# Vchitect/Latte

Hardware: AMD Instinct MI355X
Metric: denoising steps/sec (higher is better)
Workload: dtype f16; 1 GPU; Latte-XL/2 FaceForensics (uncond) 16x256x256 -> latents 16x4x32x32, DDIM on the '250' respacing, random-init weights; per_gpu_batch=8, global_batch=8, parallelism=dp1 (independent samples)

## Files before the change

### include/latte_amd_debug.h

```cpp
#ifndef LATTE_AMD_DEBUG_H_
#define LATTE_AMD_DEBUG_H_
#include <stdint.h>
#ifdef __cplusplus
extern "C" {
#endif

int latte_debug_gemm(const void* A, const void* W, const float* bias, void* out, const float* gate, int M, int N,
                     int K, int gate_stride, int rows_per_sample, int epi, int dtype, int variant, void* stream);
int latte_debug_gemm_gelu(const void* A, const void* W, const float* bias, void* out, void* aux, int M, int N, int K, int epi, int dtype,
                          void* stream);
int latte_debug_gemm_lo8(const void* A, const void* W, const void* A8, const void* W8, const float* bias, void* out, const float* gate,
                         int M, int N, int K, int gate_stride, int rows_per_sample, int epi, int dtype, void* stream);
int latte_debug_pack_w8(const void* w, void* out8, int64_t n, int dtype, void* stream);
int latte_debug_pack_w4(const void* w, void* out4, void* out_scale, int N, int K, int dtype, void* stream);
int latte_debug_ln_modulate_split4(const float* x, void* y, void* y4, void* y4s, const float* shift, const float* scale, int mod_stride, int M,
                                   int D, int rows_per_sample, int dtype, void* stream);
int latte_debug_gemm_lo4(const void* A, const void* W, const void* A4, const void* A4s, const void* W4, const void* W4s, const float* bias,
                         void* out, const float* gate, int M, int N, int K, int gate_stride, int rows_per_sample, int epi, int dtype,
                         void* stream);
int latte_debug_ln_modulate_split8(const float* x, void* y, void* y8, const float* shift, const float* scale, int mod_stride, int M, int D,
                                   int rows_per_sample, int dtype, void* stream);
int latte_debug_qkv_attention_split8(const void* xn, const void* w, const float* bias, void* out, void* out8, int B, int F, int T, int D,
                                     int heads, int mode, int dtype, void* stream);
int latte_debug_gemm_choice(int M, int N, int K, int epi);
int latte_debug_qkv_attention_fusable(int D, int heads, int F, int T, int mode, int64_t rows);
int latte_debug_gemm_tn_plan(int M, int N, int K, int* rows_per_split);
int latte_debug_attention(const void* qkv, void* out, int num_seq, int L, int heads, int hd, int U,
                          int64_t sample_stride, int64_t seq_stride, int64_t row_stride, int dtype, void* stream);
int latte_debug_cross_attention(const void* q, int q_ld, const void* kv, const float* kbias_or_null, void* out, int num_seq, int L, int Lk,
                                int heads, int hd, int U, int64_t sample_stride, int64_t seq_stride, int64_t row_stride, int dtype,
                                void* stream);
int latte_debug_small_linear(int in_mode, const float* in, const int64_t* t, const float* W, const float* bias, const float* add_table,
                             const int64_t* add_idx, float* out, int B, int N, int K, int out_stride, void* stream);
int latte_debug_patch_embed(const float* x, const float* Wt, const float* bias, const float* pos, float* out, int BF, int C, int H, int p,
                            int D, void* stream);
int latte_debug_final_layer(const float* x, const float* shift, const float* scale, int mod_stride, const float* Wt, const float* bias,
                            float* out, int M, int D, int rows_per_sample, int T, int p, int Cout, int H, void* stream);
int latte_debug_text_proj(const float* text, const float* W, const float* bias, float* out, int B, int N, int K, void* stream);
int latte_debug_gated_split_reduce(float* x, const float* ws, int splits, int64_t stride, const float* bias, const float* gate,
                                   int gate_stride, int rows_per_sample, int M, int N, void* stream);
int latte_debug_adaln_single(const float* tables, const float* head_table, const float* t6, const float* temb, float* mod, int B, int nblk,
                             int D, void* stream);
int latte_debug_cond_rows(const float* temb, const float* ytab, const int64_t* y, float* out, int n_steps, int bu, int D, void* stream);
int latte_debug_mask_bias(const float* mask, float* bias, int64_t n, void* stream);
int latte_debug_t2v_linear_step(float* x, float* x_in, const float* model_out, const float* h1, const float* h2, const float* h3,
                                const float* noise, float* hist_write, int b, int C, int Cout, int F, int hw, float scale, float m_x,
                                float m_eps, float c_x, float c0, float c1, float c2, float c3, float c_noise, float in_scale_next,
                                int push, void* stream);
int latte_debug_attention_split8(const void* qkv, void* out, void* out8, int num_seq, int L, int heads, int hd, int U, int64_t sample_stride,
                                 int64_t seq_stride, int64_t row_stride, int dtype, void* stream);
int latte_debug_qkv_attention(const void* xn, const void* w, const float* bias, void* out, void* dbg_qkv, int B, int F, int T,
                              int D, int heads, int mode, int flags, int dtype, void* stream);
int latte_debug_qkv_attention_trace(const void* xn, const void* w, const float* bias, void* out, void* dbg_qkv, long long* trace,
                                    int B, int F, int T, int D, int heads, int mode, int flags, int dtype, void* stream);
int latte_debug_attention_bwd(const void* qkv, const void* o, const void* dout, void* dqkv, float* stats, int num_seq, int L,
                              int heads, int hd, int U, int64_t sample_stride, int64_t seq_stride, int64_t row_stride, int dtype,
                              void* stream);
int latte_debug_gemm_tn(const void* dY, const void* X, float* dW, float* workspace, int64_t workspace_floats, int M, int N, int K,
                        int dtype, void* stream);
int latte_debug_gemm_tn_colsum(const void* dY, const void* X, float* dW, float* colsum, float* workspace, int64_t workspace_floats,
                               int M, int N, int K, int dtype, void* stream);
int latte_debug_ln_modulate(float* x, void* y, const float* shift, const float* scale, int mod_stride, int M, int D,
                            int rows_per_sample, const float* temp_embed, int T, int F, int dtype, void* stream);
int latte_debug_convert(const float* in, void* out, int64_t n, int dtype, void* stream);
int latte_debug_gated_add_ln(const float* x_in, const void* y, const float* gate, int gate_stride, float* x_out, void* xn,
                             const float* shift, const float* scale, int mod_stride, int M, int D, int rows_per_sample,
                             const float* temp_embed, int T, int F, int dtype, void* stream);
int latte_debug_ln_bwd(const void* dy, const float* x, const float* scale, int mod_stride, const float* dx_in, float* dx_out,
// ... 113 lines not shown
```

### latte_amd/_lib.py

```python
import ctypes
import os

import torch

_HERE = os.path.dirname(os.path.abspath(__file__))
LIB_PATH = os.path.join(_HERE, "lib", "liblatte_amd.so")

c_int, c_i64, c_f32, c_void, c_char = ctypes.c_int, ctypes.c_int64, ctypes.c_float, ctypes.c_void_p, ctypes.c_char_p
c_u64 = ctypes.c_uint64


class LatteError(RuntimeError):
    pass


class ModelConfig(ctypes.Structure):
    _fields_ = [(n, c_int) for n in ("input_size", "patch_size", "in_channels", "hidden_size", "depth", "num_heads",
                                     "mlp_hidden", "num_frames", "num_classes", "learn_sigma", "extras",
                                     "compute_dtype")]


class T2VConfig(ctypes.Structure):
    _fields_ = [(n, c_int) for n in ("num_attention_heads", "attention_head_dim", "in_channels", "out_channels", "num_layers",
                                     "sample_size", "patch_size", "cross_attention_dim", "caption_channels", "video_length",
# ... 110 lines not shown
    "latte_debug_t5_embed": (c_int, [c_void, c_void, c_void, c_int, c_int, c_int, c_void]),
    "latte_debug_t5_rmsnorm": (c_int, [c_void, c_void, c_void, c_void, c_void, c_int, c_int, c_f32, c_void]),
    "latte_debug_t5_bucket": (c_int, [c_int, c_int, c_int]),
    "latte_debug_t5_bias_table": (c_int, [c_void, c_int, c_int, c_int, c_int, c_void, c_void]),
    "latte_debug_t5_attention": (c_int, [c_void, c_void, c_void, c_void, c_void, c_int, c_int, c_int, c_int, c_void]),
    "latte_debug_t5_gated_act": (c_int, [c_void, c_void, c_void, c_int, c_int, c_void]),
    "latte_debug_t5_pack": (c_int, [c_void, c_void, c_void, c_i64, c_void]),
    "latte_debug_t5_proj_splits": (c_int, [c_int, c_int]),
    "latte_debug_t5_proj": (c_int, [c_void, c_void, c_void, c_void, c_void, c_void, c_int, c_int, c_int, c_void]),
    "latte_debug_gemm_lo8": (c_int, [c_void, c_void, c_void, c_void, c_void, c_void, c_void, c_int, c_int, c_int, c_int, c_int, c_int,
                                     c_int, c_void]),
    "latte_debug_attention_split8": (c_int, [c_void, c_void, c_void, c_int, c_int, c_int, c_int, c_int, c_i64, c_i64, c_i64, c_int, c_void]),
    "latte_debug_pack_w4": (c_int, [c_void, c_void, c_void, c_int, c_int, c_int, c_void]),
    "latte_debug_ln_modulate_split4": (c_int, [c_void, c_void, c_void, c_void, c_void, c_void, c_int, c_int, c_int, c_int, c_int, c_void]),
    "latte_debug_gemm_lo4": (c_int, [c_void, c_void, c_void, c_void, c_void, c_void, c_void, c_void, c_void, c_int, c_int, c_int, c_int, c_int,
                                     c_int, c_int, c_void]),
    "latte_debug_pack_w8": (c_int, [c_void, c_void, c_i64, c_int, c_void]),
    "latte_debug_ln_modulate_split8": (c_int, [c_void, c_void, c_void, c_void, c_void, c_int, c_int, c_int, c_int, c_int, c_void]),
    "latte_debug_qkv_attention_split8": (c_int, [c_void, c_void, c_void, c_void, c_void, c_int, c_int, c_int, c_int, c_int, c_int, c_int,
                                                 c_void]),
    "latte_debug_gemm": (c_int, [c_void, c_void, c_void, c_void, c_void, c_int, c_int, c_int, c_int, c_int, c_int,
                                 c_int, c_int, c_void]),
    "latte_debug_gemm_gelu": (c_int, [c_void, c_void, c_void, c_void, c_void, c_int, c_int, c_int, c_int, c_int, c_void]),
    "latte_debug_gemm_choice": (c_int, [c_int, c_int, c_int, c_int]),
    "latte_debug_qkv_attention_fusable": (c_int, [c_int, c_int, c_int, c_int, c_int, c_i64]),
    "latte_debug_gemm_tn_plan": (c_int, [c_int, c_int, c_int, ctypes.POINTER(c_int)]),
    "latte_debug_attention": (c_int, [c_void, c_void, c_int, c_int, c_int, c_int, c_int, c_i64, c_i64, c_i64, c_int,
                                      c_void]),
    "latte_debug_cross_attention": (c_int, [c_void, c_int, c_void, c_void, c_void, c_int, c_int, c_int, c_int, c_int, c_int, c_i64, c_i64,
                                            c_i64, c_int, c_void]),
    "latte_debug_small_linear": (c_int, [c_int, c_void, c_void, c_void, c_void, c_void, c_void, c_void, c_int, c_int, c_int, c_int,
                                         c_void]),
    "latte_debug_patch_embed": (c_int, [c_void, c_void, c_void, c_void, c_void, c_int, c_int, c_int, c_int, c_int, c_void]),
    "latte_debug_final_layer": (c_int, [c_void, c_void, c_void, c_int, c_void, c_void, c_void, c_int, c_int, c_int, c_int, c_int, c_int,
                                        c_int, c_void]),
    "latte_debug_text_proj": (c_int, [c_void, c_void, c_void, c_void, c_int, c_int, c_int, c_void]),
    "latte_debug_gated_split_reduce": (c_int, [c_void, c_void, c_int, c_i64, c_void, c_void, c_int, c_int, c_int, c_int, c_void]),
    "latte_debug_adaln_single": (c_int, [c_void, c_void, c_void, c_void, c_void, c_int, c_int, c_int, c_void]),
    "latte_debug_cond_rows": (c_int, [c_void, c_void, c_void, c_void, c_int, c_int, c_int, c_void]),
    "latte_debug_mask_bias": (c_int, [c_void, c_void, c_i64, c_void]),
    "latte_debug_t2v_linear_step": (c_int, [c_void] * 8 + [c_int] * 5 + [c_f32] * 10 + [c_int, c_void]),
    "latte_debug_qkv_attention": (c_int, [c_void, c_void, c_void, c_void, c_void, c_int, c_int, c_int, c_int, c_int, c_int, c_int,
                                          c_int, c_void]),
    "latte_debug_qkv_attention_trace": (c_int, [c_void, c_void, c_void, c_void, c_void, c_void, c_int, c_int, c_int, c_int, c_int,
                                                c_int, c_int, c_int, c_void]),
    "latte_debug_attention_bwd": (c_int, [c_void, c_void, c_void, c_void, c_void, c_int, c_int, c_int, c_int, c_int, c_i64, c_i64, c_i64,
                                          c_int, c_void]),
    "latte_debug_gemm_tn": (c_int, [c_void, c_void, c_void, c_void, c_i64, c_int, c_int, c_int, c_int, c_void]),
    "latte_debug_gemm_tn_colsum": (c_int, [c_void, c_void, c_void, c_void, c_void, c_i64, c_int, c_int, c_int, c_int, c_void]),
    "latte_debug_ln_modulate": (c_int, [c_void, c_void, c_void, c_void, c_int, c_int, c_int, c_int, c_void, c_int,
                                        c_int, c_int, c_void]),
    "latte_debug_convert": (c_int, [c_void, c_void, c_i64, c_int, c_void]),
    "latte_debug_gated_add_ln": (c_int, [c_void, c_void, c_void, c_int, c_void, c_void, c_void, c_void, c_int, c_int, c_int, c_int,
                                         c_void, c_int, c_int, c_int, c_void]),
    "latte_debug_ln_bwd": (c_int, [c_void, c_void, c_void, c_int, c_void, c_void, c_void, c_void, c_int, c_int, c_int, c_int, c_void,
                                   c_void, c_int, c_void, c_void, c_void, c_i64, c_int, c_void]),
    "latte_debug_gate_bwd": (c_int, [c_void, c_void, c_void, c_int, c_void, c_void, c_i64, c_void, c_int, c_int, c_int, c_int, c_int,
                                     c_int, c_void]),
    "latte_debug_split_reduce": (c_int, [c_void, c_int, c_i64, c_i64, c_void, c_int, c_void, c_void]),
    "latte_debug_colsum_half": (c_int, [c_void, c_int, c_int, c_void, c_i64, c_void, c_int, c_int, c_void, c_void]),
    "latte_debug_rows_sum": (c_int, [c_void, c_int, c_i64, c_int, c_void, c_int, c_void, c_void]),
    "latte_debug_naive_gemm": (c_int, [c_void, c_i64, c_i64, c_void, c_i64, c_i64, c_void, c_i64, c_i64, c_int, c_int, c_int, c_f32,
                                       c_int, c_int, c_void, c_i64, c_void, c_void]),
    "latte_debug_embedding_bwd": (c_int, [c_void, c_void, c_void, c_int, c_int, c_void, c_void]),
    "latte_debug_silu_bwd": (c_int, [c_void, c_void, c_void, c_i64, c_int, c_void]),
    "latte_debug_sumsq_blocks": (c_int, []),
# ... 125 lines not shown
```

### latte_amd/csrc/common.h

```cpp
#pragma once
#include <hip/hip_runtime.h>
#include <stdint.h>
#include <atomic>
#include <string>
#include <vector>

#include "../../include/latte_amd.h"

struct latte_schedule {
  int num_timesteps = 0;
  std::vector<int64_t> timestep_map;
  std::vector<double> betas, alphas_cumprod, alphas_cumprod_prev, sqrt_recip_alphas_cumprod,
      sqrt_recipm1_alphas_cumprod, posterior_variance, posterior_log_variance_clipped, posterior_mean_coef1,
      posterior_mean_coef2, log_betas, sqrt_alphas_cumprod, sqrt_one_minus_alphas_cumprod;
  int mean_type = 0;
  int var_type = 0;
  mutable float* dev_tables = nullptr;
  mutable int dev_tables_device = -1;
};
enum DevTable : int { DT_SQRT_AC = 0, DT_SQRT_1MAC, DT_COEF1, DT_COEF2, DT_POST_LOGVAR, DT_LOG_BETAS, DT_SQRT_RECIP, DT_SQRT_RECIPM1,
                      DT_FIXED_LOGVAR, LATTE_NUM_DEV_TABLES };

extern "C" int schedule_device_tables(const latte_schedule_t* s, const float** out, hipStream_t st);

// ... 101 lines not shown
int launch_attention(const AttnArgs& a, int dtype, hipStream_t st);
int launch_cross_attention(const AttnArgs& a, int dtype, hipStream_t st);

struct QkvAttnArgs {
  const half_t* xn;
  const half_t* w;
  const float* bias;
  half_t* out;
  half_t* dbg_qkv;
  long long* dbg_trace;
  int B, F, T, D, heads, hd;
  int mode;
  float scale;
  int flags;
  int out_split;
  unsigned char* out8;
};
bool qkv_attention_fusable(int D, int heads, int hd, int F, int T, int mode, int64_t rows);
int launch_qkv_attention(const QkvAttnArgs& a, int dtype, hipStream_t st);

int launch_ln_modulate_split4(const float* x_in, half_t* y, unsigned char* y4, unsigned char* y4s, const float* shift, const float* scale,
                              int mod_stride, int M, int D, int rows_per_sample, int dtype, hipStream_t st);
int launch_ln_modulate(const float* x_in, float* x_rw, half_t* y, const float* shift, const float* scale,
                       int mod_stride, int M, int D, int rows_per_sample, const float* temp_embed, int T,
                       int F, int dtype, hipStream_t st, int split = 0,
                       unsigned char* y8 = nullptr);
int launch_pack_w8(const half_t* in, unsigned char* out, int64_t n, int dtype, hipStream_t st);
enum SmallIn : int { IN_PLAIN = 0, IN_SILU = 1, IN_TFREQ = 2 };
int launch_small_linear(int in_mode, const float* in, const int64_t* t, const float* W, const float* bias,
                        const float* add_table, const int64_t* add_idx, float* out, int B, int N, int K,
                        int out_stride, hipStream_t st);
int launch_patch_embed(const float* x, const float* Wt , const float* bias, const float* pos,
                       float* out, int BF, int C, int H, int p, int D, hipStream_t st);
int launch_final_layer(const float* x, const float* shift, const float* scale, int mod_stride,
                       const float* Wt , const float* bias, float* out, int M, int D,
                       int rows_per_sample, int T, int p, int Cout, int H, hipStream_t st);
int launch_cond_rows(const float* temb, const float* ytab, const int64_t* y, float* out, int n_steps, int bu, int D,
                     hipStream_t st);
int launch_text_proj(const float* text, const float* W, const float* bias, float* out, int B, int N, int K, hipStream_t st);
int launch_iota(int64_t* p, int n, hipStream_t st);
int launch_gated_split_reduce(float* x, const float* ws, int splits, size_t stride, const float* bias, const float* gate,
                              int gate_stride, int rows_per_sample, int M, int N, hipStream_t st);
int launch_silu_rows(const float* in, float* out, size_t n, hipStream_t st);
int launch_adaln_single(const float* tables , const float* head_table , const float* t6 ,
                        const float* temb , float* mod, int B, int nblk, int D, hipStream_t st);
int launch_permute_cf(const float* in, float* out, int B, int C, int F, int hw, int to_bfc, hipStream_t st);
int launch_fill_f32(float* p, float v, size_t n, hipStream_t st);
enum DebugChoice { DBG_ATTN_VARIANT = 0, DBG_XATTN_FLASH, DBG_TN_KERNEL, DBG_TN_WN, DBG_ATTN_BWD_TILES, DBG_CONV_KERNEL, DBG_VAE_SPLIT, DBG_NUM_CHOICES };
int debug_choice(DebugChoice c);
int set_debug_choice(const char* name, int value);

int launch_scale_f32(float* p, float s, size_t n, hipStream_t st);
int launch_scale_f32_dev(float* p, const float* s_dev, int inverse, size_t n, hipStream_t st);
int launch_t2v_guided_ddim(float* x, const float* model_out, int b, int C, int Cout, int F, int hw, float scale, float c1, float c2,
                           float c3, float c4, hipStream_t st);
struct T2VLinearStep {
  float scale, m_x, m_eps, c_x, c0, c1, c2, c3, c_noise, in_scale_next;
  int push;
};
int launch_t2v_guided_linear_step(float* x, float* x_in, const float* model_out, const float* h1, const float* h2, const float* h3,
                                  const float* noise, float* hw, int b, int C, int Cout, int F, int HW, const T2VLinearStep& s,
                                  hipStream_t st);
int launch_mask_bias(const float* mask, float* bias, size_t n, hipStream_t st);
int launch_cfg_combine(float* out, int half_batch, int F, int Cout, int HW, float cfg_scale, hipStream_t st);
int launch_convert_f32_to_h16(const float* in, half_t* out, int64_t n, int dtype, hipStream_t st);
int launch_pack_w4(const half_t* in, unsigned char* out4, unsigned char* out_scale, int N, int K, int dtype, hipStream_t st);
// ... 145 lines not shown
```

### latte_amd/csrc/debug.hip

```cpp
#include "../../include/latte_amd_debug.h"
#include "common.h"

namespace {
typedef __attribute__((ext_vector_type(4))) __bf16 bf16x4;
__global__ void tr16_probe_kernel(uint16_t* out) {
  __shared__ __attribute__((aligned(16))) uint16_t lds[512];
  for (int i = threadIdx.x; i < 512; i += 64) lds[i] = (uint16_t)i;
  __syncthreads();
  const int lane = threadIdx.x;
  auto p = (__attribute__((address_space(3))) bf16x4*)((__attribute__((address_space(3))) char*)lds + 8 * lane);
  bf16x4 v = __builtin_amdgcn_ds_read_tr16_b64_v4bf16(p);
  typedef __attribute__((ext_vector_type(4))) unsigned short u16x4;
  u16x4 u = __builtin_bit_cast(u16x4, v);
  for (int j = 0; j < 4; ++j) out[lane * 4 + j] = u[j];
}

typedef __attribute__((address_space(3))) void lds_void_t;
__global__ void __launch_bounds__(512) dma_probe_kernel(const char* src, long long* out, int mode, int reps) {
  extern __shared__ __attribute__((aligned(16))) char smem[];
  const int lane = threadIdx.x & 63, wave = __builtin_amdgcn_readfirstlane(threadIdx.x >> 6);
  const __amdgpu_buffer_rsrc_t rs = __builtin_amdgcn_make_buffer_rsrc((void*)src, 0, 1u << 30, 0x00020000);
  char* my = smem + wave * 16384;
  const unsigned base = ((blockIdx.x & 63) * 8 + wave) * 16384u;
  long long t_issue = 0, t_all = 0;
// ... 200 lines not shown
  a.D = heads * hd; a.U = U; a.sample_stride = sample_stride; a.seq_stride = seq_stride; a.row_stride = row_stride;
  a.scale = 1.0f / sqrtf((float)hd);
  return launch_attention(a, dtype, (hipStream_t)stream);
}

int latte_debug_cross_attention(const void* q, int q_ld, const void* kv, const float* kbias_or_null, void* out, int num_seq, int L, int Lk,
                                int heads, int hd, int U, int64_t sample_stride, int64_t seq_stride, int64_t row_stride, int dtype,
                                void* stream) {
  if (!q || !kv || !out || num_seq < 1 || L < 1 || Lk < 1 || heads < 1 || U < 1 || sample_stride < 0 || seq_stride < 0 || row_stride < 1)
    return fail(LATTE_ERR_INVALID, "cross_attention: bad arguments");
  if (hd != 64 && hd != 72) return fail(LATTE_ERR_INVALID, "cross_attention: head_dim must be 64 or 72");
  if (q_ld < heads * hd || q_ld % 8) return fail(LATTE_ERR_INVALID, "cross_attention: need q_ld >= heads * hd and q_ld % 8 == 0");
  AttnArgs a{};
  a.qkv = (const half_t*)q; a.out = (half_t*)out; a.num_seq = num_seq; a.L = L; a.heads = heads; a.hd = hd; a.D = heads * hd; a.U = U;
  a.sample_stride = sample_stride; a.seq_stride = seq_stride; a.row_stride = row_stride; a.scale = 1.0f / sqrtf((float)hd);
  a.kv = (const half_t*)kv; a.kbias = kbias_or_null; a.Lk = Lk; a.q_ld = q_ld;
  return launch_cross_attention(a, dtype, (hipStream_t)stream);
}

int latte_debug_small_linear(int in_mode, const float* in, const int64_t* t, const float* W, const float* bias, const float* add_table,
                             const int64_t* add_idx, float* out, int B, int N, int K, int out_stride, void* stream) {
  if (!W || !bias || !out || B < 1 || N < 1 || K < 1 || out_stride < N || (in_mode == IN_TFREQ ? !t : !in) || (add_table && !add_idx))
    return fail(LATTE_ERR_INVALID, "small_linear: bad arguments (out_stride >= N, t in mode 2, in otherwise, add_idx with add_table)");
  return launch_small_linear(in_mode, in, t, W, bias, add_table, add_idx, out, B, N, K, out_stride, (hipStream_t)stream);
}

int latte_debug_patch_embed(const float* x, const float* Wt, const float* bias, const float* pos, float* out, int BF, int C, int H, int p,
                            int D, void* stream) {
  if (!x || !Wt || !bias || !pos || !out || BF < 1 || C < 1 || H < 1 || p < 1 || D < 1)
    return fail(LATTE_ERR_INVALID, "patch_embed: bad arguments");
  if (D % 128) return fail(LATTE_ERR_INVALID, "patch_embed: D must be a multiple of 128");
  if (H % p) return fail(LATTE_ERR_INVALID, "patch_embed: H must be a multiple of the patch size");
  if ((int64_t)16 * C * p * p * (int64_t)sizeof(float) > 65536)
    return fail(LATTE_ERR_INVALID, "patch_embed: 16 tokens x C p p floats exceed the default dynamic LDS limit (64 KiB)");
  return launch_patch_embed(x, Wt, bias, pos, out, BF, C, H, p, D, (hipStream_t)stream);
}

int latte_debug_final_layer(const float* x, const float* shift, const float* scale, int mod_stride, const float* Wt, const float* bias,
                            float* out, int M, int D, int rows_per_sample, int T, int p, int Cout, int H, void* stream) {
  if (!x || !shift || !scale || !Wt || !bias || !out || M < 1 || D < 1 || T < 1 || p < 1 || Cout < 1 || H < 1 || mod_stride < 0)
    return fail(LATTE_ERR_INVALID, "final_layer: bad arguments");
  if (D % 128) return fail(LATTE_ERR_INVALID, "final_layer: D must be a multiple of 128");
  if (H % p) return fail(LATTE_ERR_INVALID, "final_layer: H must be a multiple of the patch size");
  if (rows_per_sample <= 0) return fail(LATTE_ERR_INVALID, "final_layer: rows_per_sample must be positive");
  if (T != (H / p) * (H / p) || M % T || mod_stride % 2)
    return fail(LATTE_ERR_INVALID, "final_layer: need T == (H / p)^2, whole frames (M % T == 0) and an even mod_stride");
  return launch_final_layer(x, shift, scale, mod_stride, Wt, bias, out, M, D, rows_per_sample, T, p, Cout, H, (hipStream_t)stream);
}

int latte_debug_text_proj(const float* text, const float* W, const float* bias, float* out, int B, int N, int K, void* stream) {
  if (!text || !W || !bias || !out || B < 1 || N < 1 || K < 1) return fail(LATTE_ERR_INVALID, "text_proj: bad arguments");
  return launch_text_proj(text, W, bias, out, B, N, K, (hipStream_t)stream);
}

int latte_debug_gated_split_reduce(float* x, const float* ws, int splits, int64_t stride, const float* bias, const float* gate,
                                   int gate_stride, int rows_per_sample, int M, int N, void* stream) {
  if (!x || !ws || !bias || !gate || M < 1 || N < 1 || rows_per_sample <= 0 || gate_stride < 0 || gate_stride % 4 || stride % 4 ||
      stride < (int64_t)M * N)
    return fail(LATTE_ERR_INVALID, "gated_split_reduce: need rows_per_sample > 0, stride >= M * N, stride and gate_stride multiples of 4");
  return launch_gated_split_reduce(x, ws, splits, (size_t)stride, bias, gate, gate_stride, rows_per_sample, M, N, (hipStream_t)stream);
}

int latte_debug_adaln_single(const float* tables, const float* head_table, const float* t6, const float* temb, float* mod, int B, int nblk,
                             int D, void* stream) {
  if (!tables || !head_table || !t6 || !temb || !mod || B < 1 || nblk < 1 || D < 1) return fail(LATTE_ERR_INVALID, "adaln_single: bad arguments");
  return launch_adaln_single(tables, head_table, t6, temb, mod, B, nblk, D, (hipStream_t)stream);
}

// ... 575 lines not shown
```

### latte_amd/csrc/pointwise.hip

```cpp
#include "common.h"
#include "mfma_util.h"

namespace latte {
namespace {

template <int NCH, int DT, bool ADD_TE, int SPLIT = 0>
__global__ void __launch_bounds__(256) ln_modulate_kernel(const float* __restrict__ x_in, float* x_rw,
                                                          half_t* __restrict__ y, const float* __restrict__ shift,
                                                          const float* __restrict__ scale, int mod_stride, int M,
                                                          int rows_per_sample, const float* __restrict__ te, int T,
                                                          int F, unsigned char* __restrict__ y8 = nullptr,
                                                          unsigned char* __restrict__ y4s = nullptr) {
  constexpr int D = NCH * 128;
  constexpr int NT = NCH * 32;
  constexpr int NQ = (NT + 63) / 64;
  const int lane = threadIdx.x & 63;
  const int row = blockIdx.x * 4 + (threadIdx.x >> 6);
  if (row >= M) return;
  const float4* xr = (const float4*)(x_in + (size_t)row * D);
  auto has = [&](int c) -> bool { return (c + 1) * 64 <= NT || c * 64 + lane < NT; };
  float4 v[NQ];
#pragma unroll
  for (int c = 0; c < NQ; ++c) v[c] = has(c) ? xr[c * 64 + lane] : make_float4(0.f, 0.f, 0.f, 0.f);
  const int smp = row / rows_per_sample;
// ... 120 lines not shown
            const int fi = k < half ? k : k - half;
            const float freq = expf((-9.210340371976184f * (float)fi) / (float)half);
            const float arg = tv * freq;
            e[u] = k < half ? cosf(arg) : sinf(arg);
          }
          acc = fmaf(e[0], w[c].x, acc);
          acc = fmaf(e[1], w[c].y, acc);
        }
      }
    } else {
      const float2* ir = (const float2*)(in + (size_t)b * K);
#pragma unroll
      for (int c = 0; c < SL_MAXCH; ++c) {
        if (c < nch) {
          float2 a = ir[c * 64 + lane];
          if constexpr (IN_MODE == IN_SILU) {
            a.x = silu(a.x);
            a.y = silu(a.y);
          }
          acc = fmaf(a.x, w[c].x, acc);
          acc = fmaf(a.y, w[c].y, acc);
        }
      }
    }
    acc = wave_sum(acc);
    if (lane == 0) {
      float r = acc + bn;
      if (add_table != nullptr) r += add_table[(size_t)add_idx[b] * N + n];
      out[(size_t)b * out_stride + n] = r;
    }
  }
}

constexpr int PE_TOK = 16;
__global__ void __launch_bounds__(128) patch_embed_kernel(const float* __restrict__ x, const float* __restrict__ Wt,
                                                          const float* __restrict__ bias, const float* __restrict__ pos,
                                                          float* __restrict__ out, int ntok, int C, int H, int p, int D) {
  extern __shared__ float xs[];
  const int K = C * p * p;
  const int G = H / p, T = G * G;
  const int tok0 = blockIdx.x * PE_TOK;
  for (int i = threadIdx.x; i < PE_TOK * K; i += 128) {
    const int tk = i / K, k = i % K;
    const int n = tok0 + tk;
    float v = 0.f;
    if (n < ntok) {
      const int bf = n / T, tt = n % T;
      const int hp = tt / G, wp = tt % G;
      const int c = k / (p * p), ii = (k / p) % p, jj = k % p;
      v = x[(((size_t)bf * C + c) * H + hp * p + ii) * H + wp * p + jj];
    }
    xs[i] = v;
  }
  __syncthreads();
  const int tg = threadIdx.x >> 5, q = threadIdx.x & 31;
  const int d = blockIdx.y * 128 + q * 4;
  float4 acc[4];
#pragma unroll
  for (int tk = 0; tk < 4; ++tk) acc[tk] = make_float4(0.f, 0.f, 0.f, 0.f);
  for (int k = 0; k < K; ++k) {
    const float4 w = *(const float4*)(Wt + (size_t)k * D + d);
#pragma unroll
    for (int tk = 0; tk < 4; ++tk) {
      const float xv = xs[(tg * 4 + tk) * K + k];
      acc[tk].x = fmaf(xv, w.x, acc[tk].x);
      acc[tk].y = fmaf(xv, w.y, acc[tk].y);
      acc[tk].z = fmaf(xv, w.z, acc[tk].z);
      acc[tk].w = fmaf(xv, w.w, acc[tk].w);
    }
  }
  const float4 bv = *(const float4*)(bias + d);
#pragma unroll
  for (int tk = 0; tk < 4; ++tk) {
    const int n = tok0 + tg * 4 + tk;
    if (n < ntok) {
      const float4 pv = *(const float4*)(pos + (size_t)(n % T) * D + d);
      *(float4*)(out + (size_t)n * D + d) = make_float4(acc[tk].x + bv.x + pv.x, acc[tk].y + bv.y + pv.y, acc[tk].z + bv.z + pv.z,
                                                        acc[tk].w + bv.w + pv.w);
    }
  }
}

constexpr int FL_ROWS = 8;
template <int NCH>
__global__ void __launch_bounds__(256) final_layer_kernel(const float* __restrict__ x, const float* __restrict__ shift,
                                                          const float* __restrict__ scale, int mod_stride,
                                                          const float* __restrict__ Wt, const float* __restrict__ bias,
                                                          float* __restrict__ out, int M, int rows_per_sample, int T,
                                                          int p, int Cout, int H) {
  constexpr int D = NCH * 128;
  extern __shared__ float xs[];
  const int lane = threadIdx.x & 63, wave = threadIdx.x >> 6;
  const int row0 = blockIdx.x * FL_ROWS;
  for (int rr = wave; rr < FL_ROWS; rr += 4) {
    const int row = row0 + rr;
    float2* xo = (float2*)(xs + rr * D);
    if (row >= M) {
#pragma unroll
      for (int c = 0; c < NCH; ++c) xo[c * 64 + lane] = make_float2(0.f, 0.f);
      continue;
    }
    const float2* xr = (const float2*)(x + (size_t)row * D);
    float2 v[NCH];
    float s = 0.f;
#pragma unroll
    for (int c = 0; c < NCH; ++c) {
      v[c] = xr[c * 64 + lane];
      s += v[c].x + v[c].y;
    }
    const float mean = wave_sum(s) * (1.0f / D);
    float q = 0.f;
// ... 699 lines not shown
      else                                                                                                     \
        hipLaunchKernelGGL((ln_modulate_kernel<NCH, LATTE_DTYPE_F16, false>), grid, block, 0, st, x_in, x_rw, y, \
                           shift, scale, mod_stride, M, rows_per_sample, temp_embed, T, F);                    \
    }                                                                                                          \
  } while (0)
  LATTE_NCH_SWITCH(D, LN_LAUNCH)
#undef LN_LAUNCH
  LATTE_HIP(hipGetLastError());
  return LATTE_OK;
}

int launch_small_linear(int in_mode, const float* in, const int64_t* t, const float* W, const float* bias,
                        const float* add_table, const int64_t* add_idx, float* out, int B, int N, int K,
                        int out_stride, hipStream_t st) {
  if (K % 128 != 0 || K > 128 * SL_MAXCH) return fail(LATTE_ERR_INVALID, "small_linear: need K % 128 == 0 and K <= 1152");
  dim3 grid((N + 3) / 4), block(256);
  switch (in_mode) {
    case IN_PLAIN:
      hipLaunchKernelGGL(small_linear_kernel<IN_PLAIN>, grid, block, 0, st, in, t, W, bias, add_table, add_idx, out, B, N, K, out_stride);
      break;
    case IN_SILU:
      hipLaunchKernelGGL(small_linear_kernel<IN_SILU>, grid, block, 0, st, in, t, W, bias, add_table, add_idx, out, B, N, K, out_stride);
      break;
    case IN_TFREQ:
      hipLaunchKernelGGL(small_linear_kernel<IN_TFREQ>, grid, block, 0, st, in, t, W, bias, add_table, add_idx, out, B, N, K, out_stride);
      break;
    default:
      return fail(LATTE_ERR_INVALID, "small_linear: bad input mode");
  }
  LATTE_HIP(hipGetLastError());
  return LATTE_OK;
}

int launch_patch_embed(const float* x, const float* Wt, const float* bias, const float* pos, float* out, int BF,
                       int C, int H, int p, int D, hipStream_t st) {
  const int G = H / p, ntok = BF * G * G, K = C * p * p;
  dim3 grid((ntok + PE_TOK - 1) / PE_TOK, D / 128), block(128);
  hipLaunchKernelGGL(patch_embed_kernel, grid, block, PE_TOK * K * sizeof(float), st, x, Wt, bias, pos, out, ntok, C, H, p, D);
  LATTE_HIP(hipGetLastError());
  return LATTE_OK;
}

int launch_final_layer(const float* x, const float* shift, const float* scale, int mod_stride, const float* Wt,
                       const float* bias, float* out, int M, int D, int rows_per_sample, int T, int p, int Cout,
                       int H, hipStream_t st) {
  dim3 grid((M + FL_ROWS - 1) / FL_ROWS), block(256);
  const size_t lds = (size_t)FL_ROWS * D * sizeof(float);
#define FL_LAUNCH(NCH)                                                                                       \
  hipLaunchKernelGGL(final_layer_kernel<NCH>, grid, block, lds, st, x, shift, scale, mod_stride, Wt, bias, out, M, \
                     rows_per_sample, T, p, Cout, H)
  LATTE_NCH_SWITCH(D, FL_LAUNCH)
#undef FL_LAUNCH
  LATTE_HIP(hipGetLastError());
  return LATTE_OK;
}

int launch_cond_rows(const float* temb, const float* ytab, const int64_t* y, float* out, int n_steps, int bu, int D,
                     hipStream_t st) {
  const size_t n = (size_t)n_steps * bu * D;
  hipLaunchKernelGGL(cond_rows_kernel, dim3(grid_for(n, 256)), dim3(256), 0, st, temb, ytab, y, out, n_steps, bu, D);
  LATTE_HIP(hipGetLastError());
  return LATTE_OK;
}

int launch_text_proj(const float* text, const float* W, const float* bias, float* out, int B, int N, int K,
                     hipStream_t st) {
  if (K % 128) return fail(LATTE_ERR_INVALID, "text_proj: K must be a multiple of 128");
  hipLaunchKernelGGL(text_proj_kernel, dim3((N + 3) / 4), dim3(256), 0, st, text, W, bias, out, B, N, K);
  LATTE_HIP(hipGetLastError());
  return LATTE_OK;
}

int launch_gated_split_reduce(float* x, const float* ws, int splits, size_t stride, const float* bias, const float* gate,
// ... 140 lines not shown
```

Baseline: 260.0 sample-steps/s.

## Restructure patch embed kernel with LDS-staged weights and persistent grid; add fused LN variant

Rewrites the patch-embedding kernel. The weight matrix (or chunks of it) is staged in LDS, and each wave computes four tokens across the full hidden width. A persistent grid of about two blocks per CU is used, with prefetch of the next block's pixels. It also adds an optional variant that applies LayerNorm plus adaLN modulation and writes f16/bf16 activations, so the first block's separate norm pass could be removed, but only a debug entry point calls it here. The aim is to cut repeated global weight reads and launch fragmentation, at the cost of heavy LDS use and more register pressure.

```diff
diff --git a/include/latte_amd_debug.h b/include/latte_amd_debug.h
--- a/include/latte_amd_debug.h
+++ b/include/latte_amd_debug.h
@@ -34,6 +34,9 @@
                              const int64_t* add_idx, float* out, int B, int N, int K, int out_stride, void* stream);
 int latte_debug_patch_embed(const float* x, const float* Wt, const float* bias, const float* pos, float* out, int BF, int C, int H, int p,
                             int D, void* stream);
+int latte_debug_patch_embed_ln(const float* x, const float* Wt, const float* bias, const float* pos, float* out, void* xn, const float* shift,
+                               const float* scale, int mod_stride, int rows_per_sample, int BF, int C, int H, int p, int D, int dtype,
+                               void* stream);
 int latte_debug_final_layer(const float* x, const float* shift, const float* scale, int mod_stride, const float* Wt, const float* bias,
                             float* out, int M, int D, int rows_per_sample, int T, int p, int Cout, int H, void* stream);
 int latte_debug_text_proj(const float* text, const float* W, const float* bias, float* out, int B, int N, int K, void* stream);
diff --git a/latte_amd/_lib.py b/latte_amd/_lib.py
--- a/latte_amd/_lib.py
+++ b/latte_amd/_lib.py
@@ -166,6 +166,8 @@
     "latte_debug_small_linear": (c_int, [c_int, c_void, c_void, c_void, c_void, c_void, c_void, c_void, c_int, c_int, c_int, c_int,
                                          c_void]),
     "latte_debug_patch_embed": (c_int, [c_void, c_void, c_void, c_void, c_void, c_int, c_int, c_int, c_int, c_int, c_void]),
+    "latte_debug_patch_embed_ln": (c_int, [c_void, c_void, c_void, c_void, c_void, c_void, c_void, c_void, c_int, c_int, c_int, c_int, c_int,
+                                           c_int, c_int, c_int, c_void]),
     "latte_debug_final_layer": (c_int, [c_void, c_void, c_void, c_int, c_void, c_void, c_void, c_int, c_int, c_int, c_int, c_int, c_int,
                                         c_int, c_void]),
     "latte_debug_text_proj": (c_int, [c_void, c_void, c_void, c_void, c_int, c_int, c_int, c_void]),
diff --git a/latte_amd/csrc/common.h b/latte_amd/csrc/common.h
--- a/latte_amd/csrc/common.h
+++ b/latte_amd/csrc/common.h
@@ -157,6 +157,9 @@
                         int out_stride, hipStream_t st);
 int launch_patch_embed(const float* x, const float* Wt , const float* bias, const float* pos,
                        float* out, int BF, int C, int H, int p, int D, hipStream_t st);
+int launch_patch_embed_ln(const float* x, const float* Wt, const float* bias, const float* pos, float* out, half_t* xn,
+                          const float* shift, const float* scale, int mod_stride, int rows_per_sample, int BF, int C, int H, int p,
+                          int D, int dtype, hipStream_t st);
 int launch_final_layer(const float* x, const float* shift, const float* scale, int mod_stride,
                        const float* Wt , const float* bias, float* out, int M, int D,
                        int rows_per_sample, int T, int p, int Cout, int H, hipStream_t st);
diff --git a/latte_amd/csrc/debug.hip b/latte_amd/csrc/debug.hip
--- a/latte_amd/csrc/debug.hip
+++ b/latte_amd/csrc/debug.hip
@@ -256,8 +256,23 @@
   if (D % 128) return fail(LATTE_ERR_INVALID, "patch_embed: D must be a multiple of 128");
   if (H % p) return fail(LATTE_ERR_INVALID, "patch_embed: H must be a multiple of the patch size");
   if ((int64_t)16 * C * p * p * (int64_t)sizeof(float) > 65536)
-    return fail(LATTE_ERR_INVALID, "patch_embed: 16 tokens x C p p floats exceed the default dynamic LDS limit (64 KiB)");
+    return fail(LATTE_ERR_INVALID, "patch_embed: 16 C p p floats exceed 64 KiB");
   return launch_patch_embed(x, Wt, bias, pos, out, BF, C, H, p, D, (hipStream_t)stream);
+}
+
+int latte_debug_patch_embed_ln(const float* x, const float* Wt, const float* bias, const float* pos, float* out, void* xn, const float* shift,
+                               const float* scale, int mod_stride, int rows_per_sample, int BF, int C, int H, int p, int D, int dtype,
+                               void* stream) {
+  if (!x || !Wt || !bias || !pos || !out || !xn || !shift || !scale || BF < 1 || C < 1 || H < 1 || p < 1 || D < 1 || mod_stride < 0 ||
+      rows_per_sample < 1 || (dtype != LATTE_DTYPE_F16 && dtype != LATTE_DTYPE_BF16))
+    return fail(LATTE_ERR_INVALID, "patch_embed_ln: bad arguments");
+  if (D % 128) return fail(LATTE_ERR_INVALID, "patch_embed_ln: D must be a multiple of 128");
+  if (H % p) return fail(LATTE_ERR_INVALID, "patch_embed_ln: H must be a multiple of the patch size");
+  if (mod_stride % 4) return fail(LATTE_ERR_INVALID, "patch_embed_ln: mod_stride must be a multiple of 4 (16-byte loads)");
+  if ((int64_t)16 * C * p * p * (int64_t)sizeof(float) > 65536)
+    return fail(LATTE_ERR_INVALID, "patch_embed_ln: 16 C p p floats exceed 64 KiB, as patch_embed");
+  return launch_patch_embed_ln(x, Wt, bias, pos, out, (half_t*)xn, shift, scale, mod_stride, rows_per_sample, BF, C, H, p, D, dtype,
+                               (hipStream_t)stream);
 }
 
 int latte_debug_final_layer(const float* x, const float* shift, const float* scale, int mod_stride, const float* Wt, const float* bias,
diff --git a/latte_amd/csrc/pointwise.hip b/latte_amd/csrc/pointwise.hip
--- a/latte_amd/csrc/pointwise.hip
+++ b/latte_amd/csrc/pointwise.hip
@@ -176,51 +176,169 @@
   }
 }
 
-constexpr int PE_TOK = 16;
-__global__ void __launch_bounds__(128) patch_embed_kernel(const float* __restrict__ x, const float* __restrict__ Wt,
-                                                          const float* __restrict__ bias, const float* __restrict__ pos,
-                                                          float* __restrict__ out, int ntok, int C, int H, int p, int D) {
-  extern __shared__ float xs[];
+constexpr int PE_TOK = 16, PE_R = 4, PE_PF = 1;
+constexpr int PE_W_BYTES = 72 * 1024;
+inline int pe_kc(int K, int D) { const int kc = PE_W_BYTES / (D * (int)sizeof(float)); return K < kc ? K : kc; }
+inline int pe_lds_bytes(int kc, int D) { return (kc * D + PE_TOK * kc) * (int)sizeof(float); }
+constexpr int PE_LDS_MAX = PE_W_BYTES + PE_TOK * (PE_W_BYTES / (128 * 4)) * 4;
+template <int NCH, bool LN, int DT>
+__global__ void __launch_bounds__(256, 2) patch_embed_kernel(const float* __restrict__ x, const float* __restrict__ Wt,
+                                                             const float* __restrict__ bias, const float* __restrict__ pos,
+                                                             float* __restrict__ out, half_t* __restrict__ xn,
+                                                             const float* __restrict__ shift, const float* __restrict__ scale,
+                                                             int mod_stride, int rows_per_sample, int ntok, int C, int H, int p,
+                                                             int KC) {
+  constexpr int D = NCH * 128;
+  constexpr int NT = NCH * 32;
+  constexpr int NQ = (NT + 63) / 64;
+  extern __shared__ float pe_lds[];
+  float4* wl = (float4*)pe_lds;
+  const int lane = threadIdx.x & 63, wave = threadIdx.x >> 6;
+  float* px = pe_lds + (size_t)KC * D + wave * PE_R * KC;
   const int K = C * p * p;
   const int G = H / p, T = G * G;
-  const int tok0 = blockIdx.x * PE_TOK;
-  for (int i = threadIdx.x; i < PE_TOK * K; i += 128) {
-    const int tk = i / K, k = i % K;
-    const int n = tok0 + tk;
-    float v = 0.f;
-    if (n < ntok) {
-      const int bf = n / T, tt = n % T;
-      const int hp = tt / G, wp = tt % G;
-      const int c = k / (p * p), ii = (k / p) % p, jj = k % p;
-      v = x[(((size_t)bf * C + c) * H + hp * p + ii) * H + wp * p + jj];
-    }
-    xs[i] = v;
-  }
-  __syncthreads();
-  const int tg = threadIdx.x >> 5, q = threadIdx.x & 31;
-  const int d = blockIdx.y * 128 + q * 4;
-  float4 acc[4];
-#pragma unroll
-  for (int tk = 0; tk < 4; ++tk) acc[tk] = make_float4(0.f, 0.f, 0.f, 0.f);
-  for (int k = 0; k < K; ++k) {
-    const float4 w = *(const float4*)(Wt + (size_t)k * D + d);
-#pragma unroll
-    for (int tk = 0; tk < 4; ++tk) {
-      const float xv = xs[(tg * 4 + tk) * K + k];
-      acc[tk].x = fmaf(xv, w.x, acc[tk].x);
-      acc[tk].y = fmaf(xv, w.y, acc[tk].y);
-      acc[tk].z = fmaf(xv, w.z, acc[tk].z);
-      acc[tk].w = fmaf(xv, w.w, acc[tk].w);
-    }
-  }
-  const float4 bv = *(const float4*)(bias + d);
-#pragma unroll
-  for (int tk = 0; tk < 4; ++tk) {
-    const int n = tok0 + tg * 4 + tk;
-    if (n < ntok) {
-      const float4 pv = *(const float4*)(pos + (size_t)(n % T) * D + d);
-      *(float4*)(out + (size_t)n * D + d) = make_float4(acc[tk].x + bv.x + pv.x, acc[tk].y + bv.y + pv.y, acc[tk].z + bv.z + pv.z,
-                                                        acc[tk].w + bv.w + pv.w);
+  const bool whole = KC >= K;
+  auto has = [&](int c) -> bool { return (c + 1) * 64 <= NT || c * 64 + lane < NT; };
+  auto pixel = [&](int n, int k) -> float {
+    if (n >= ntok) return 0.f;
+    const int bf = n / T, tt = n % T;
+    const int hp = tt / G, wp = tt % G;
+    const int ch = k / (p * p), ii = (k / p) % p, jj = k % p;
+    return x[(((size_t)bf * C + ch) * H + hp * p + ii) * H + wp * p + jj];
+  };
+  const bool ahead = whole && PE_R * K <= 64 * PE_PF;
+  float pn[PE_PF];
+  auto request = [&](int blk) {
+#pragma unroll
+    for (int u = 0; u < PE_PF; ++u) {
+      const int i = lane + 64 * u;
+      pn[u] = i < PE_R * K ? pixel(blk * PE_TOK + wave * PE_R + i / K, i % K) : 0.f;
+    }
+  };
+  float4 bv[NQ];
+#pragma unroll
+  for (int c = 0; c < NQ; ++c) bv[c] = has(c) ? ((const float4*)bias)[c * 64 + lane] : make_float4(0.f, 0.f, 0.f, 0.f);
+  const int nblk = (ntok + PE_TOK - 1) / PE_TOK;
+  if (ahead && (int)blockIdx.x < nblk) request(blockIdx.x);
+  if (whole) {
+    const float4* wg = (const float4*)Wt;
+    for (int i = threadIdx.x; i < K * NT; i += 256) wl[i] = wg[i];
+    __syncthreads();
+  }
+  for (int blk = blockIdx.x; blk < nblk; blk += gridDim.x) {
+    const int tok0 = blk * PE_TOK + wave * PE_R;
+    float4 acc[PE_R][NQ];
+#pragma unroll
+    for (int r = 0; r < PE_R; ++r)
+#pragma unroll
+      for (int c = 0; c < NQ; ++c) acc[r][c] = make_float4(0.f, 0.f, 0.f, 0.f);
+    for (int k0 = 0; k0 < K; k0 += KC) {
+      const int kc = K - k0 < KC ? K - k0 : KC;
+      if (!whole) {
+        __syncthreads();
+        const float4* wg = (const float4*)(Wt + (size_t)k0 * D);
+        for (int i = threadIdx.x; i < kc * NT; i += 256) wl[i] = wg[i];
+      }
+      if (ahead) {
+#pragma unroll
+        for (int u = 0; u < PE_PF; ++u) {
+          const int i = lane + 64 * u;
+          if (i < PE_R * K) px[(i / K) * KC + i % K] = pn[u];
+        }
+        if (blk + (int)gridDim.x < nblk) request(blk + gridDim.x);
+      } else {
+        for (int i = lane; i < PE_R * kc; i += 64) px[(i / kc) * KC + i % kc] = pixel(tok0 + i / kc, k0 + i % kc);
+      }
+      if (whole) {
+        __builtin_amdgcn_fence(__ATOMIC_RELEASE, "wavefront");
+        __builtin_amdgcn_wave_barrier();
+        __builtin_amdgcn_fence(__ATOMIC_ACQUIRE, "wavefront");
+      } else {
+        __syncthreads();
+      }
+      for (int k = 0; k < kc; ++k) {
+        float xv[PE_R];
+#pragma unroll
+        for (int r = 0; r < PE_R; ++r) xv[r] = px[r * KC + k];
+#pragma unroll
+        for (int c = 0; c < NQ; ++c) {
+          const float4 w = wl[k * NT + (has(c) ? c * 64 + lane : 0)];
+#pragma unroll
+          for (int r = 0; r < PE_R; ++r) {
+            acc[r][c].x = fmaf(xv[r], w.x, acc[r][c].x);
+            acc[r][c].y = fmaf(xv[r], w.y, acc[r][c].y);
+            acc[r][c].z = fmaf(xv[r], w.z, acc[r][c].z);
+            acc[r][c].w = fmaf(xv[r], w.w, acc[r][c].w);
+          }
+        }
+      }
+    }
+    int rowc[PE_R];
+#pragma unroll
+    for (int r = 0; r < PE_R; ++r) rowc[r] = tok0 + r < ntok ? tok0 + r : ntok - 1;
+    float4 pv[PE_R][NQ];
+#pragma unroll
+    for (int r = 0; r < PE_R; ++r) {
+      const float4* pr = (const float4*)(pos + (size_t)(rowc[r] % T) * D);
+#pragma unroll
+      for (int c = 0; c < NQ; ++c) pv[r][c] = has(c) ? pr[c * 64 + lane] : make_float4(0.f, 0.f, 0.f, 0.f);
+    }
+    float4 (&v)[PE_R][NQ] = acc;
+#pragma unroll
+    for (int r = 0; r < PE_R; ++r) {
+      float4* orow = (float4*)(out + (size_t)rowc[r] * D);
+      const bool live = tok0 + r < ntok;
+#pragma unroll
+      for (int c = 0; c < NQ; ++c) {
+        if (has(c)) {
+          v[r][c] = make_float4(acc[r][c].x + bv[c].x + pv[r][c].x, acc[r][c].y + bv[c].y + pv[r][c].y,
+                                acc[r][c].z + bv[c].z + pv[r][c].z, acc[r][c].w + bv[c].w + pv[r][c].w);
+          if (live) orow[c * 64 + lane] = v[r][c];
+        } else {
+          v[r][c] = make_float4(0.f, 0.f, 0.f, 0.f);
+        }
+      }
+    }
+    if constexpr (LN) {
+      float mean[PE_R], rstd[PE_R];
+#pragma unroll
+      for (int r = 0; r < PE_R; ++r) {
+        float s = 0.f;
+#pragma unroll
+        for (int c = 0; c < NQ; ++c) s += (v[r][c].x + v[r][c].y) + (v[r][c].z + v[r][c].w);
+        mean[r] = wave_sum(s) * (1.0f / D);
+      }
+#pragma unroll
+      for (int r = 0; r < PE_R; ++r) {
+        float q = 0.f;
+#pragma unroll
+        for (int c = 0; c < NQ; ++c) {
+          if (has(c)) {
+            const float a = v[r][c].x - mean[r], b = v[r][c].y - mean[r], d = v[r][c].z - mean[r], e = v[r][c].w - mean[r];
+            q += (a * a + b * b) + (d * d + e * e);
+          }
+        }
+        rstd[r] = 1.0f / sqrtf(wave_sum(q) * (1.0f / D) + 1e-6f);
+      }
+#pragma unroll
+      for (int r = 0; r < PE_R; ++r) {
+        const int smp = rowc[r] / rows_per_sample;
+        const float4* sh = (const float4*)(shift + (size_t)smp * mod_stride);
+        const float4* sc = (const float4*)(scale + (size_t)smp * mod_stride);
+        u32x2* yr = (u32x2*)(xn + (size_t)rowc[r] * D);
+        const bool live = tok0 + r < ntok;
+#pragma unroll
+        for (int c = 0; c < NQ; ++c) {
+          if (has(c)) {
+            const float4 a = sh[c * 64 + lane], b = sc[c * 64 + lane];
+            const float o0 = (v[r][c].x - mean[r]) * rstd[r] * (1.0f + b.x) + a.x;
+            const float o1 = (v[r][c].y - mean[r]) * rstd[r] * (1.0f + b.y) + a.y;
+            const float o2 = (v[r][c].z - mean[r]) * rstd[r] * (1.0f + b.z) + a.z;
+            const float o3 = (v[r][c].w - mean[r]) * rstd[r] * (1.0f + b.w) + a.w;
+            if (live) yr[c * 64 + lane] = (u32x2){pack2<DT>(o0, o1), pack2<DT>(o2, o3)};
+          }
+        }
+      }
     }
   }
 }
@@ -986,13 +1104,60 @@
   return LATTE_OK;
 }
 
+static int device_cus(int* cus) {
+  static std::atomic<int> known[64];
+  int dev = 0;
+  LATTE_HIP(hipGetDevice(&dev));
+  int n = known[dev & 63].load(std::memory_order_relaxed);
+  if (n <= 0) {
+    LATTE_HIP(hipDeviceGetAttribute(&n, hipDeviceAttributeMultiprocessorCount, dev));
+    if (n <= 0) return fail(LATTE_ERR_HIP, "no compute units reported for the device");
+    known[dev & 63].store(n, std::memory_order_relaxed);
+  }
+  *cus = n;
+  return LATTE_OK;
+}
+
+template <bool LN>
+static int patch_embed_launch(const float* x, const float* Wt, const float* bias, const float* pos, float* out, half_t* xn,
+                              const float* shift, const float* scale, int mod_stride, int rows_per_sample, int BF, int C, int H, int p,
+                              int D, int dtype, hipStream_t st) {
+  if (D % 128 != 0) return fail(LATTE_ERR_INVALID, "patch_embed: D % 128 != 0");
+  const int G = H / p, ntok = BF * G * G, K = C * p * p;
+  int cus = 0;
+  if (int rc = device_cus(&cus)) return rc;
+  const int nblk = (ntok + PE_TOK - 1) / PE_TOK;
+  dim3 grid(nblk < 2 * cus ? nblk : 2 * cus), block(256);
+  const int kc = pe_kc(K, D), lds = pe_lds_bytes(kc, D);
+  int rc = LATTE_OK;
+#define PE_LAUNCH(NCH)                                                                                                     \
+  do {                                                                                                                     \
+    if constexpr (LN) {                                                                                                    \
+      if (dtype == LATTE_DTYPE_BF16) {                                                                                     \
+        rc = launch_lds_max<patch_embed_kernel<NCH, true, LATTE_DTYPE_BF16>>(grid, block, PE_LDS_MAX, lds, st, x, Wt, bias, pos, out, xn, \
+                                                                             shift, scale, mod_stride, rows_per_sample, ntok, C, H, p, kc); \
+        break;                                                                                                             \
+      }                                                                                                                    \
+    }                                                                                                                      \
+    rc = launch_lds_max<patch_embed_kernel<NCH, LN, LATTE_DTYPE_F16>>(grid, block, PE_LDS_MAX, lds, st, x, Wt, bias, pos, out, xn, \
+                                                                      shift, scale, mod_stride, rows_per_sample, ntok, C, H, p, kc); \
+  } while (0)
+  LATTE_NCH_SWITCH(D, PE_LAUNCH)
+#undef PE_LAUNCH
+  return rc;
+}
+
 int launch_patch_embed(const float* x, const float* Wt, const float* bias, const float* pos, float* out, int BF,
                        int C, int H, int p, int D, hipStream_t st) {
-  const int G = H / p, ntok = BF * G * G, K = C * p * p;
-  dim3 grid((ntok + PE_TOK - 1) / PE_TOK, D / 128), block(128);
-  hipLaunchKernelGGL(patch_embed_kernel, grid, block, PE_TOK * K * sizeof(float), st, x, Wt, bias, pos, out, ntok, C, H, p, D);
-  LATTE_HIP(hipGetLastError());
-  return LATTE_OK;
+  return patch_embed_launch<false>(x, Wt, bias, pos, out, nullptr, nullptr, nullptr, 0, 1, BF, C, H, p, D, LATTE_DTYPE_F16, st);
+}
+
+int launch_patch_embed_ln(const float* x, const float* Wt, const float* bias, const float* pos, float* out, half_t* xn,
+                          const float* shift, const float* scale, int mod_stride, int rows_per_sample, int BF, int C, int H, int p,
+                          int D, int dtype, hipStream_t st) {
+  if (!xn || !shift || !scale || rows_per_sample <= 0)
+    return fail(LATTE_ERR_INVALID, "patch_embed_ln: needs xn, shift, scale and a positive rows_per_sample");
+  return patch_embed_launch<true>(x, Wt, bias, pos, out, xn, shift, scale, mod_stride, rows_per_sample, BF, C, H, p, D, dtype, st);
 }
 
 int launch_final_layer(const float* x, const float* shift, const float* scale, int mod_stride, const float* Wt,
```

Result: no change. 260.0 sample-steps/s (median of 2 runs) (-0.0%).
